# megapose6d/megapose6d

Measured on AMD Instinct MI355X. Metric: pose-hypotheses/sec (render+coarse+refine), 640×480, megapose-1.0-RGB, higher is better.
Workload: dtype f32 (results of fp32 arithmetic; the convolutions' multiplications run on the bf16 MFMA as EXACT piece products of the fp32 operands, fp32 accumulate)

## Files before the change

### include/mp_engine.h

```cpp
#ifndef MP_ENGINE_H
#define MP_ENGINE_H

#include <stddef.h>
#include <stdint.h>

#ifdef __cplusplus
extern "C" {
#endif

typedef void* mp_stream;

#define MP_OK 0
#define MP_ERR_INVALID (-22)
#define MP_ERR_NOMEM (-12)
#define MP_ERR_HIP (-5)

int mp_version(void);
const char* mp_last_error(void);
int mp_profile_begin(void);
int mp_profile_end(void);
int mp_profile_active(void);
int mp_profile_query(int idx, char* name, int name_len, int64_t* launches, double* total_ms, double* total_flops,
                     double* total_bytes);
int mp_profile_query_ex(int idx, char* name, int name_len, int64_t* launches, double* total_ms, double* total_flops,
// ... 110 lines not shown
const char* mp_conv2d_kernel_name(const mp_conv_desc* desc);

size_t mp_conv_bf16x9_packed_bytes(int Cin_p, int Cout, int KH, int KW);
int mp_conv_bf16x9_pack_weights(const float* h_w_oihw, int Cout, int Cin, int KH, int KW, int Cin_p, const float* h_scale ,
                                void* h_packed);
int mp_conv2d_bf16x9_nhwc(const mp_conv_desc* desc, const void* d_w_pieces, mp_stream stream);

size_t mp_conv_wino_packed_floats(int Cin_p, int Cout);
int mp_conv_wino_pack_weights(const float* h_w_oi33, int Cout, int Cin, int Cin_p, const float* h_scale , float* h_packed);
int mp_conv_wino_eligible(const mp_conv_desc* desc, int n_cu);
int mp_conv3x3_wino_nhwc(const mp_conv_desc* desc, const float* d_u, mp_stream stream);

size_t mp_conv_wino_bf16_packed_bytes(int Cin_p, int Cout);
int mp_conv_wino_bf16_pack_weights(const float* h_w_oi33, int Cout, int Cin, int Cin_p, const float* h_scale , void* h_packed);
int mp_conv3x3_wino_bf16_nhwc(const mp_conv_desc* desc, const void* d_u_pieces, mp_stream stream);

int mp_xrec_elements(int n_f32, int n_u8);
int mp_conv_stem_supported(int KS, int n_f32, int n_u8);
size_t mp_conv_stem_packed_bytes(int KS, int n_f32, int n_u8, int Cout);
int mp_conv_stem_pack_weights(const float* h_w_oihw, int Cout, int Cin, int KS, int n_f32, const float* h_scale ,
                              void* h_packed);
int mp_conv_stem_pack_weights_mask(const float* h_w_oihw, int Cout, int Cin, int KS, uint32_t f32_mask, const float* h_scale,
                                   void* h_packed);
int mp_conv_stem_xrec(const mp_conv_desc* desc, const void* d_packed, int n_f32, mp_stream stream);
int mp_conv_stem_xrec_pool(const mp_conv_desc* desc, const void* d_packed, int n_f32, float* d_ypool, int pool_border, mp_stream stream);

int mp_conv_stem_sparse_chunks(int KS, int n_f32, int n_u8);
size_t mp_conv_stem_sparse_packed_bytes(int KS, int n_f32, int n_u8, int Cout);
int mp_conv_stem_pack_weights_sparse(const float* h_w_oihw, int Cout, int Cin, int KS, int n_f32, const float* h_scale, void* h_packed);
int mp_conv_stem_xrec_sparse(const mp_conv_desc* desc, const void* d_packed, const void* d_packed_sparse, int n_f32,
// ... 151 lines not shown
```

### megapose6d_amd/_lib.py

```python
from __future__ import annotations

import ctypes as C
import os
from pathlib import Path

_HERE = Path(__file__).resolve().parent
LIB_PATH = _HERE / "libmp_engine.so"


class EngineError(RuntimeError):
    pass


class MeshDesc(C.Structure):
    _fields_ = [
        ("h_vertices", C.c_void_p),
        ("h_normals", C.c_void_p),
        ("h_colors", C.c_void_p),
        ("h_faces", C.c_void_p),
        ("n_vertices", C.c_int32),
        ("n_faces", C.c_int32),
    ]


# ... 85 lines not shown
    "mp_conv_pack_weights": (_i, [_vp, _i, _i, _i, _i, _i, _vp, _vp]),
    "mp_conv2d_nhwc": (_i, [C.POINTER(ConvDesc), _vp]),
    "mp_conv2d_plan": (_i, [C.POINTER(ConvDesc), _i, C.POINTER(C.c_int32)]),
    "mp_conv_bf16x9_packed_bytes": (_sz, [_i, _i, _i, _i]),
    "mp_conv_bf16x9_pack_weights": (_i, [_vp, _i, _i, _i, _i, _i, _vp, _vp]),
    "mp_conv2d_bf16x9_nhwc": (_i, [C.POINTER(ConvDesc), _vp, _vp]),
    "mp_conv2d_kernel_name": (C.c_char_p, [C.POINTER(ConvDesc)]),
    "mp_conv_wino_packed_floats": (_sz, [_i, _i]),
    "mp_conv_wino_pack_weights": (_i, [_vp, _i, _i, _i, _vp, _vp]),
    "mp_conv_wino_eligible": (_i, [C.POINTER(ConvDesc), _i]),
    "mp_conv3x3_wino_nhwc": (_i, [C.POINTER(ConvDesc), _vp, _vp]),
    "mp_conv_wino_stats": (_i, [C.POINTER(C.c_double), C.POINTER(C.c_double), _i]),
    "mp_conv_wino_bf16_packed_bytes": (_sz, [_i, _i]),
    "mp_conv_wino_bf16_pack_weights": (_i, [_vp, _i, _i, _i, _vp, _vp]),
    "mp_conv3x3_wino_bf16_nhwc": (_i, [C.POINTER(ConvDesc), _vp, _vp]),
    "mp_conv_wino_bf16_stats": (_i, [C.POINTER(C.c_double), C.POINTER(C.c_double), _i]),
    "mp_conv_wino_bf16_clock": (_i, [C.POINTER(C.c_double), C.POINTER(C.c_double), _i]),
    "mp_conv_wino_bf16_phases": (_i, [C.POINTER(C.c_double), C.POINTER(C.c_double)]),
    "mp_conv_wino_bf16_telemetry": (_i, [_i]),
    "mp_xrec_elements": (_i, [_i, _i]),
    "mp_conv_stem_supported": (_i, [_i, _i, _i]),
    "mp_conv_stem_packed_bytes": (_sz, [_i, _i, _i, _i]),
    "mp_conv_stem_pack_weights": (_i, [_vp, _i, _i, _i, _i, _vp, _vp]),
    "mp_conv_stem_pack_weights_mask": (_i, [_vp, _i, _i, _i, _u32, _vp, _vp]),
    "mp_conv_stem_sparse_chunks": (_i, [_i, _i, _i]),
    "mp_conv_stem_sparse_packed_bytes": (_sz, [_i, _i, _i, _i]),
    "mp_conv_stem_pack_weights_sparse": (_i, [_vp, _i, _i, _i, _i, _vp, _vp]),
    "mp_conv_stem_xrec_sparse": (_i, [C.POINTER(ConvDesc), _vp, _vp, _i, _vp, _vp, _i, _vp]),
    "mp_conv_stem_bg_stats": (_i, [C.POINTER(C.c_double), C.POINTER(C.c_double), _i]),
    "mp_conv_stem_xrec": (_i, [C.POINTER(ConvDesc), _vp, _i, _vp]),
# ... 81 lines not shown
```

### megapose6d_amd/csrc/backbone.hip

```cpp
#include <cmath>
#include <cstdlib>
#include <map>
#include <mutex>
#include <string>
#include <vector>

#include "common.h"

namespace mp {

struct ConvLayer {
  int Cin, Cin_p, Cout, K, stride, pad;
  float* d_w = nullptr;
  float* d_u = nullptr;
  void* d_ub = nullptr;
  void* d_wb = nullptr;
  float* d_b = nullptr;
};

struct BnAct {
  float* d_scale = nullptr;
  float* d_shift = nullptr;
};

// ... 113 lines not shown
    if (rc) return rc;
  }
  return MP_OK;
}

int make_bnact(mp_backbone* bb, const StateMap& sm, const std::string& bnkey, int C, BnAct* a) {
  std::vector<float> scale, shift;
  int rc = bn_affine(sm, bnkey, C, scale, shift);
  if (rc) return rc;
  rc = upload(bb, scale, &a->d_scale);
  if (rc) return rc;
  return upload(bb, shift, &a->d_shift);
}

constexpr size_t SPLITK_WS_FLOATS = 12u << 20;

int run_conv(const mp_backbone* bb, const ConvLayer& L, const float* x, int N, int H, int W, int in_border, float* y, int out_border,
             const float* res, int relu, float* y_act, const BnAct* act, hipStream_t s, float* splitk_ws = nullptr, bool x_f16 = false) {
  mp_conv_desc d;
  memset(&d, 0, sizeof(d));
  d.x_f16 = x_f16 ? 1 : 0;
  d.d_x = x; d.N = N; d.H = H; d.W = W; d.C = L.Cin_p; d.c_real = L.Cin; d.in_border = in_border;
  d.d_w = L.d_w; d.d_bias = L.d_b; d.Cout = L.Cout; d.KH = L.K; d.KW = L.K; d.stride = L.stride; d.pad = L.pad;
  d.d_y = y; d.out_border = out_border; d.d_residual = res; d.relu = relu;
  d.d_y_act = y_act;
  if (y_act) { d.d_act_scale = act->d_scale; d.d_act_shift = act->d_shift; }
  d.d_splitk_ws = splitk_ws;
  d.splitk_ws_floats = splitk_ws ? (int64_t)SPLITK_WS_FLOATS : 0;
  if ((L.d_u || L.d_ub || L.d_wb) && !x_f16) {
    static int n_cu = 0, n_cu_dev = -1, lds_ok = 0;
    int dev = 0;
    (void)hipGetDevice(&dev);
    if (n_cu_dev != dev) {
      if (hipDeviceGetAttribute(&n_cu, hipDeviceAttributeMultiprocessorCount, dev) != hipSuccess || n_cu <= 0) n_cu = 256;
      int lds = 0;
      lds_ok = hipDeviceGetAttribute(&lds, hipDeviceAttributeMaxSharedMemoryPerBlock, dev) == hipSuccess && lds >= 132 * 1024;
      n_cu_dev = dev;
    }
    if ((L.d_u || L.d_ub) && lds_ok && mp_conv_wino_eligible(&d, n_cu))
      return L.d_ub ? mp_conv3x3_wino_bf16_nhwc(&d, L.d_ub, s) : mp_conv3x3_wino_nhwc(&d, L.d_u, s);
    if (L.d_wb) {
      int32_t plan[5] = {0, 1, 0, 0, 0};
      const int rc = mp_conv2d_plan(&d, n_cu, plan);
      if (rc) return rc;
      if (plan[0] != 1) return mp_conv2d_bf16x9_nhwc(&d, L.d_wb, s);
    }
  }
  return mp_conv2d_nhwc(&d, s);
}

inline size_t align_up(size_t v, size_t a) { return (v + a - 1) / a * a; }
inline size_t buf_floats(int N, int H, int W, int C) { return (size_t)N * (H + 2) * (W + 2) * C + (size_t)(W + 3) * C + 64; }

struct Geometry {
  int h1, w1;
// ... 2 lines not shown

Geometry geometry(const mp_backbone* bb, int h, int w) {
  Geometry g;
  g.h1 = (h + 2 * bb->stem.pad - bb->stem.K) / 2 + 1;
  g.w1 = (w + 2 * bb->stem.pad - bb->stem.K) / 2 + 1;
  g.hs[0] = (g.h1 + 2 - 3) / 2 + 1;
  g.ws[0] = (g.w1 + 2 - 3) / 2 + 1;
  for (int s = 1; s < 4; ++s) {
    g.hs[s] = (g.hs[s - 1] + 2 - 3) / 2 + 1;
    g.ws[s] = (g.ws[s - 1] + 2 - 3) / 2 + 1;
  }
  return g;
}


}

extern "C" int mp_backbone_create(int kind, int c_in, int head_kind, int n_head_out, const mp_named_tensor* st, int n_tensors,
                                  mp_backbone** out) {
  return mp_backbone_create_wide(kind, 1, c_in, head_kind, n_head_out, st, n_tensors, out);
}

extern "C" int mp_backbone_create_wide(int kind, int width, int c_in, int head_kind, int n_head_out, const mp_named_tensor* st, int n_tensors,
                                       mp_backbone** out) {
  MP_REQUIRE(out && st && n_tensors > 0, "mp_backbone_create: bad arguments");
  MP_REQUIRE(kind >= 0 && kind <= 2, "mp_backbone_create: unknown backbone kind %d", kind);
  MP_REQUIRE(width >= 1 && width <= 8 && (width == 1 || kind != MP_BACKBONE_VANILLA_RESNET34),
             "mp_backbone_create: width multiplier %d (1..8, WideResNets only: training/pose_models_cfg.py:114-116)", width);
  MP_REQUIRE(c_in >= 1 && c_in <= 512, "mp_backbone_create: bad c_in %d", c_in);
  StateMap sm;
// ... 286 lines not shown
```

### megapose6d_amd/csrc/conv_wino_bf16.hip

```cpp
#include <atomic>
#include <cstdlib>
#include <mutex>
#include <vector>

#include "bf16x9_split.h"
#include "wino_common.h"

namespace mp {

typedef __bf16 bf16x8 __attribute__((ext_vector_type(8)));
typedef float f32x2 __attribute__((ext_vector_type(2)));


__device__ __forceinline__ unsigned pack_hi16(unsigned e1, unsigned e0) { return __builtin_amdgcn_perm(e1, e0, 0x07060302u); }

__device__ __forceinline__ float f4c(const float4& v, int c) { return c == 0 ? v.x : c == 1 ? v.y : c == 2 ? v.z : v.w; }
__device__ constexpr int WB_PA[9] = {2, 1, 2, 0, 1, 2, 0, 1, 0}, WB_PB[9] = {2, 2, 1, 2, 1, 0, 1, 0, 0};

constexpr int UB_F_BYTES = 2 * 3 * 1024;
constexpr int UB_STEP_BYTES = 16 * UB_F_BYTES;
constexpr size_t WB_LDS_BYTES = (size_t)4 * 2 * WT * 72 * sizeof(float);
static_assert(WB_LDS_BYTES >= WINO_LDS_BYTES && WB_LDS_BYTES <= 160 * 1024, "LDS budget of conv3x3_wino_bf16x9");

__device__ unsigned long long g_wb_clk[6];
#ifdef MP_WINO_PHASES
__device__ unsigned long long g_wb_phase[10];
#define WB_PHASE(K, T0) if (ph_sample) atomicAdd(&g_wb_phase[K], __builtin_readcyclecounter() - (T0));
#else
#define WB_PHASE(K, T0)
#endif

template <int DIAG, bool RES, bool ACT, bool PERSIST = false>
__global__ __launch_bounds__(256) __attribute__((amdgpu_waves_per_eu(1, 1))) void conv3x3_wino_bf16x9(WinoParams p) {
  extern __shared__ __attribute__((aligned(16))) float smem[];
  float* Vs = smem;
  int* tile_tab = (int*)(smem + 4 * 2 * WT * WCOUT);

  unsigned long long clk_start = __builtin_readcyclecounter();
  const int tid = threadIdx.x, lane = tid & 63;
#ifdef MP_WINO_PHASES
  const bool ph_sample = (blockIdx.x & 63) == 0 && threadIdx.x == 0;
#endif
  const int wave = __builtin_amdgcn_readfirstlane(tid >> 6);
  const __amdgpu_buffer_rsrc_t x_rsrc = __builtin_amdgcn_make_buffer_rsrc((void*)p.x, 0, -1, 0x00020000);
  const int row_bytes = p.Wp * p.C * 4, pix_bytes = p.C * 4;
  const int u_voff = lane * 16;
  const int ptile = tid >> 2, pc4 = tid & 3;
  float4 patch[4][4];
  int unit = (int)blockIdx.x;
  const int n_units = PERSIST ? p.n_units : (int)gridDim.x;
  int cb, tile0, x_voff;
  __amdgpu_buffer_rsrc_t u_rsrc;
#define WB_UNIT_INDICES(U)                                                                               \
  {                                                                                                      \
    const int wg_ = xcd_remap((U), n_units);                                                             \
    const int tg_ = (int)wino_fastdiv((unsigned)wg_, (unsigned)p.n_cblocks, p.mg_cb, p.sh_cb);           \
    cb = wg_ - tg_ * p.n_cblocks;                                                                        \
    tile0 = tg_ * WT;                                                                                    \
    const unsigned char* ub_ = reinterpret_cast<const unsigned char*>(p.u) + (size_t)cb * p.n_steps * UB_STEP_BYTES + (size_t)(4 * wave) * UB_F_BYTES;  \
    u_rsrc = __builtin_amdgcn_make_buffer_rsrc((void*)ub_, 0, -1, 0x00020000);                            \
    int t_ = tile0 + ptile;                                                                              \
    t_ = t_ < p.n_tiles ? t_ : p.n_tiles - 1;                                                            \
    const int r_ = (int)wino_fastdiv((unsigned)t_, (unsigned)p.tiles_x, p.mg_tx, p.sh_tx), tx_ = t_ - r_ * p.tiles_x;   \
    const int n_ = (int)wino_fastdiv((unsigned)r_, (unsigned)p.tiles_y, p.mg_ty, p.sh_ty), ty_ = r_ - n_ * p.tiles_y;   \
    const size_t pix_ = ((size_t)n_ * p.Hp + (size_t)(2 * ty_ + p.in_off)) * p.Wp + (size_t)(2 * tx_ + p.in_off);  \
    x_voff = (int)((pix_ * p.C + pc4 * 4) * sizeof(float));                                               \
  }
  float* vw = Vs + ptile * WCK + ((pc4 ^ ((ptile >> 2) & 3)) * 4);



  f32x16 acc[4][2][2];
  const int ns = p.n_steps;
  u32x4 Ua[2][3], Ub[2][3];
  u32x4 AA[2][3], AB[2][3];
  float4 raw[2][2];
  unsigned sm0, sm1, sm2, sm3;
  float sr0, sr1, sr2, sr3, sq0, sq1, sq2, sq3;
  float4 trw[4], tplane;
  if (DIAG & (7 | 32 | 64 | 128)) {
    _Pragma("unroll") for (int i = 0; i < 2; ++i)
      _Pragma("unroll") for (int q = 0; q < 3; ++q) { AA[i][q] = AB[i][q] = Ua[i][q] = Ub[i][q] = u32x4{0x3f803f80u, 0x3f803f80u, 0x3f803f80u, 0x3f803f80u}; }
    _Pragma("unroll") for (int a = 0; a < 4; ++a) { trw[a] = make_float4(0.f, 0.f, 0.f, 0.f);
      _Pragma("unroll") for (int bb = 0; bb < 4; ++bb) patch[a][bb] = make_float4(1.f, 1.f, 1.f, 1.f); }
    tplane = make_float4(0.f, 0.f, 0.f, 0.f);
    sm0 = sm1 = sm2 = sm3 = 0u; sr0 = sr1 = sr2 = sr3 = sq0 = sq1 = sq2 = sq3 = 0.f;
  }
#define WB_SB __builtin_amdgcn_sched_barrier(0);
// ... 90 lines not shown
  const int fo_lo = ((2 * (lane >> 5)) ^ fsw) * 4, fo_hi = ((2 * (lane >> 5) + 1) ^ fsw) * 4;

  float4 pnext[4][4];
#define WB_UNIT_REQUESTS() \
  _Pragma("unroll") for (int a = 0; a < 4; ++a) \
    _Pragma("unroll") for (int bb = 0; bb < 4; ++bb) { WB_LOAD_PATCH1(a, bb, 0) } \
  WB_SB \
  if (tid < WT) { \
    const int t = tile0 + tid; \
    int off = -1, bits = 0; \
    if (t < p.n_tiles) { \
      const int r = (int)wino_fastdiv((unsigned)t, (unsigned)p.tiles_x, p.mg_tx, p.sh_tx), tx = t - r * p.tiles_x; \
      const int n = (int)wino_fastdiv((unsigned)r, (unsigned)p.tiles_y, p.mg_ty, p.sh_ty), ty = r - n * p.tiles_y; \
      off = ((n * p.Hop + 2 * ty + p.out_border) * p.Wop + 2 * tx + p.out_border) * p.Cout; \
      bits = ((2 * ty + 1 < p.Ho) ? 1 : 0) | ((2 * tx + 1 < p.Wo) ? 2 : 0); \
    } \
    tile_tab[2 * tid] = off; \
    tile_tab[2 * tid + 1] = bits; \
  } \
  { \
    const u32x4 z4 = {0u, 0u, 0u, 0u}; \
    _Pragma("unroll") for (int fi = 0; fi < 4; ++fi) \
      _Pragma("unroll") for (int i = 0; i < 2; ++i) \
        _Pragma("unroll") for (int j = 0; j < 2; ++j) \
          asm volatile("s_nop 1\n\tv_mfma_f32_32x32x16_bf16 %0, %1, %1, 0" : "=a"(acc[fi][i][j]) : "v"(z4)); \
  } \
  WB_SB
#define WB_UNIT_TABLE() \
  if (tid < WT) { \
    const int t = tile0 + tid; \
    int off = -1, bits = 0; \
    if (t < p.n_tiles) { \
      const int r = (int)wino_fastdiv((unsigned)t, (unsigned)p.tiles_x, p.mg_tx, p.sh_tx), tx = t - r * p.tiles_x; \
      const int n = (int)wino_fastdiv((unsigned)r, (unsigned)p.tiles_y, p.mg_ty, p.sh_ty), ty = r - n * p.tiles_y; \
      off = ((n * p.Hop + 2 * ty + p.out_border) * p.Wop + 2 * tx + p.out_border) * p.Cout; \
      bits = ((2 * ty + 1 < p.Ho) ? 1 : 0) | ((2 * tx + 1 < p.Wo) ? 2 : 0); \
    } \
    tile_tab[2 * tid] = off; \
    tile_tab[2 * tid + 1] = bits; \
  }
  WB_UNIT_INDICES(unit)
  WB_UNIT_REQUESTS()
  for (;;) {
  _Pragma("unroll") for (int k = 0; k < 6; ++k) { WB_LOAD_U1(Ua, 0, 0, k) }
  WB_SB
  WB_PHASE(0, clk_start)
#define WB_TR_ROW(A, VW) WB_TR_T(A, 0) WB_TR_T(A, 1) WB_TR_T(A, 2) WB_TR_T(A, 3) WB_TR_P(0) WB_TR_W(A, 0, VW) WB_TR_P(1) WB_TR_W(A, 1, VW) WB_TR_P(2) WB_TR_W(A, 2, VW) WB_TR_P(3) WB_TR_W(A, 3, VW)
  WB_TR_ROW(0, vw) WB_PHASE(1, clk_start)
  WB_SB
  const int cs1 = (ns > 1 ? 1 : 0) * (WCK * 4);
#define WB_PN(K) WB_SB pnext[(K) >> 2][(K) & 3] = buf4(x_rsrc, x_voff, cs1 + ((K) >> 2) * row_bytes + ((K) & 3) * pix_bytes); WB_SB
// ... 3 lines not shown
  WB_TR_ROW_PN(1, vw, 0) WB_PN(5) WB_TR_ROW_PN(2, vw, 6) WB_TR_ROW_PN(3, vw, 11)
#undef WB_TR_ROW_PN
#undef WB_PN
  WB_PHASE(2, clk_start)
  _Pragma("unroll") for (int a = 0; a < 4; ++a)
    _Pragma("unroll") for (int bb = 0; bb < 4; ++bb) patch[a][bb] = pnext[a][bb];
  __syncthreads();
  WB_PHASE(3, clk_start)
  constexpr unsigned WOOB = 0xFFFFFFF0u;
  int2 ttab[4];
  _Pragma("unroll") for (int it = 0; it < 4; ++it) ttab[it] = *reinterpret_cast<const int2*>(tile_tab + 2 * (it * 16 + (tid >> 4)));
  WB_READ_RAW1(vr, 0, 0) WB_READ_RAW1(vr, 0, 1) WB_READ_RAW1(vr, 0, 2) WB_READ_RAW1(vr, 0, 3)
#define WB_SPLIT4(AN, I, H) WB_SP0(AN, I, H) WB_SP1(I, H) WB_SP2(AN, I, H) WB_SP3() WB_SP4(AN, I, H)
  WB_SPLIT4(AA, 0, 0) WB_SPLIT4(AA, 0, 1) WB_SPLIT4(AA, 1, 0) WB_SPLIT4(AA, 1, 1)
  WB_READ_RAW1(vr, 1, 0) WB_READ_RAW1(vr, 1, 1) WB_READ_RAW1(vr, 1, 2) WB_READ_RAW1(vr, 1, 3)
  const int n = cb * WCOUT + (tid & 15) * 4;
  unsigned voff[4][4];
  {
    const int e_row = p.Wop * p.Cout * 4, e_pix = p.Cout * 4;
    _Pragma("unroll") for (int it = 0; it < 4; ++it) {
      const int off = ttab[it].x, bits = ttab[it].y;
      const unsigned base = (unsigned)(off + n) * 4u;
      const bool t_ok = off >= 0;
      voff[it][0] = t_ok ? base : WOOB;
      voff[it][1] = (t_ok && (bits & 2)) ? base + (unsigned)e_pix : WOOB;
      voff[it][2] = (t_ok && (bits & 1)) ? base + (unsigned)e_row : WOOB;
      voff[it][3] = (t_ok && (bits & 3) == 3) ? base + (unsigned)(e_row + e_pix) : WOOB;
    }
  }
  const int out_bytes = p.out_bytes;
  const __amdgpu_buffer_rsrc_t r_res = __builtin_amdgcn_make_buffer_rsrc((void*)p.residual, 0, (RES && p.residual) ? out_bytes : 0, 0x00020000);
  u32x4 res[4][4];

#ifdef MP_WINO_PERMUTE
// ... 178 lines not shown
#undef WB_TR_W
#undef WB_TR_P
#undef WB_TR_ROW
#undef WB_TR_T
#undef WB_F4ASM
#undef WB_OP_SUB
#undef WB_OP_ADD
#undef WB_LOAD_PATCH1
#undef WB_LOAD_U1
#undef WB_SB
#undef WB_UNIT_TABLE
#undef WB_UNIT_REQUESTS
#undef WB_UNIT_INDICES
}

}

using namespace mp;

extern "C" size_t mp_conv_wino_bf16_packed_bytes(int Cin_p, int Cout) { return (size_t)(Cout / WCOUT) * (Cin_p / WCK) * UB_STEP_BYTES; }

extern "C" int mp_conv_wino_bf16_pack_weights(const float* w, int Cout, int Cin, int Cin_p, const float* scale, void* packed_bytes) {
  MP_REQUIRE(w && packed_bytes && Cin_p >= Cin && Cin_p % WCK == 0 && Cout % WCOUT == 0,
             "mp_conv_wino_bf16_pack_weights: bad arguments (Cin_p %% 16, Cout %% 64)");
  static const double G[4][3] = {{1, 0, 0}, {0.5, 0.5, 0.5}, {0.5, -0.5, 0.5}, {0, 0, 1}};
  const int n_steps = Cin_p / WCK;
  unsigned short* out = (unsigned short*)packed_bytes;
  memset(out, 0, mp_conv_wino_bf16_packed_bytes(Cin_p, Cout));
  for (int n = 0; n < Cout; ++n) {
    const double s = scale ? (double)scale[n] : 1.0;
// ... 52 lines not shown
#endif

extern "C" int mp_conv_wino_bf16_clock(double* shader_mhz, double* cycles_per_step, int reset) {
  unsigned long long h[6] = {0, 0, 0, 0, 0, 0};
  MP_CHECK_HIP(hipDeviceSynchronize());
  MP_CHECK_HIP(hipMemcpyFromSymbol(h, HIP_SYMBOL(g_wb_clk), sizeof(h)));
  if (shader_mhz) *shader_mhz = h[1] ? 100.0 * (double)h[0] / (double)h[1] : 0.0;
  if (cycles_per_step) *cycles_per_step = h[2] ? (double)h[0] / (double)h[2] : 0.0;
  if (reset) {
    const unsigned long long z[6] = {0, 0, 0, 0, 0, 0};
    MP_CHECK_HIP(hipMemcpyToSymbol(HIP_SYMBOL(g_wb_clk), z, sizeof(z)));
  }
  return MP_OK;
}

extern "C" int mp_conv3x3_wino_bf16_nhwc(const mp_conv_desc* d, const void* d_u_pieces, mp_stream stream) {
  MP_REQUIRE(d && d->d_x && d_u_pieces && (d->d_y || d->d_y_act), "mp_conv3x3_wino_bf16_nhwc: null pointer");
  MP_REQUIRE(d->KH == 3 && d->KW == 3 && d->stride == 1 && d->pad == 1, "mp_conv3x3_wino_bf16_nhwc: 3x3 / stride 1 / pad 1 only");
  MP_REQUIRE(d->C % WCK == 0 && d->Cout % WCOUT == 0 && d->in_border >= 1, "mp_conv3x3_wino_bf16_nhwc: C %% 16, Cout %% 64, in_border >= 1");
  MP_REQUIRE(!d->d_y_act || (d->d_act_scale && d->d_act_shift), "mp_conv3x3_wino_bf16_nhwc: y_act needs scale/shift");
  WinoParams p;
  p.x = d->d_x; p.u = (const float*)d_u_pieces; p.bias = d->d_bias; p.residual = d->d_residual; p.act_scale = d->d_act_scale; p.act_shift = d->d_act_shift;
  p.y = d->d_y; p.y_act = d->d_y_act;
  p.N = d->N; p.Ho = d->H; p.Wo = d->W;
  p.Hp = d->H + 2 * d->in_border; p.Wp = d->W + 2 * d->in_border; p.C = d->C;
  p.in_off = d->in_border - 1;
  p.Cout = d->Cout;
  p.Hop = d->H + 2 * d->out_border; p.Wop = d->W + 2 * d->out_border; p.out_border = d->out_border;
  p.tiles_x = (d->W + 1) / 2; p.tiles_y = (d->H + 1) / 2;
  const long n_tiles = (long)d->N * p.tiles_x * p.tiles_y;
  const long in_bytes = ((long)d->N * p.Hp + 2) * p.Wp * p.C * 4, out_elems = (long)d->N * p.Hop * p.Wop * d->Cout;
// ... 2 lines not shown
  p.n_tiles = (int)n_tiles;
  p.n_chunks = d->C / 8;
  p.n_steps = d->C / WCK;
  wino_fastdiv_make((unsigned)p.tiles_x, &p.mg_tx, &p.sh_tx);
  wino_fastdiv_make((unsigned)p.tiles_y, &p.mg_ty, &p.sh_ty);
  p.relu = d->relu;
  p.n_cblocks = d->Cout / WCOUT;
  wino_fastdiv_make((unsigned)p.n_cblocks, &p.mg_cb, &p.sh_cb);
  int dev = 0;
  MP_CHECK_HIP(hipGetDevice(&dev));
  static int attr_dev = -1;
  if (attr_dev != dev) {
#define WB_ATTR(...) MP_CHECK_HIP(hipFuncSetAttribute((const void*)conv3x3_wino_bf16x9<__VA_ARGS__>, hipFuncAttributeMaxDynamicSharedMemorySize, (int)WB_LDS_BYTES));
    WB_ATTR(0, false, false) WB_ATTR(0, true, false) WB_ATTR(0, false, true) WB_ATTR(0, true, true)
    WB_ATTR(0, false, false, true) WB_ATTR(0, true, false, true) WB_ATTR(0, false, true, true) WB_ATTR(0, true, true, true)
#ifdef MP_CONV_EXPERIMENTS
    WB_ATTR(1, true, true) WB_ATTR(2, true, true) WB_ATTR(4, true, true) WB_ATTR(7, true, true) WB_ATTR(8, true, true) WB_ATTR(16, true, true)
    WB_ATTR(32, true, true) WB_ATTR(64, true, true) WB_ATTR(128, true, true)
#endif
#undef WB_ATTR
    attr_dev = dev;
  }
  const long n_wg = ((n_tiles + WT - 1) / WT) * p.n_cblocks;
  hipStream_t s = (hipStream_t)stream;
  const double c_real = d->c_real > 0 ? d->c_real : d->C;
  const double direct = 2.0 * 9.0 * (double)d->N * d->H * d->W * c_real * d->Cout;
  const double executed = 9.0 * 2.0 * 16.0 * (double)n_tiles * c_real * d->Cout;
  {
    std::lock_guard<std::mutex> lock(g_wb_mu);
    g_wb_direct += direct;
    g_wb_executed += executed;
  }
  p.telemetry = g_wb_telemetry.load(std::memory_order_relaxed);
  ProfScope prof("conv3x3_wino_bf16x9<64t,64c>", direct, 4.0 * ((double)d->N * d->H * d->W * (d->C + d->Cout)) + 6.0 * 16.0 * d->C * d->Cout, s, executed, 2500.0);
  const dim3 grid((unsigned)n_wg), block(256);
  static const int persist_env = getenv("MP_WINO_PERSIST") ? atoi(getenv("MP_WINO_PERSIST")) : 1;
  static int n_cu = 0;
  if (!n_cu) { hipDeviceProp_t prop; MP_CHECK_HIP(hipGetDeviceProperties(&prop, dev)); n_cu = prop.multiProcessorCount; }
  p.n_units = (int)n_wg;
  bool launched = false;
#ifdef MP_CONV_EXPERIMENTS
  const int diag = getenv("MP_WINO_DIAG") ? atoi(getenv("MP_WINO_DIAG")) : 0;
#define WB_DIAG_LAUNCH(D) if (diag == D) { hipLaunchKernelGGL((conv3x3_wino_bf16x9<D, true, true>), grid, block, WB_LDS_BYTES, s, p); launched = true; }
  WB_DIAG_LAUNCH(1) WB_DIAG_LAUNCH(2) WB_DIAG_LAUNCH(4) WB_DIAG_LAUNCH(7) WB_DIAG_LAUNCH(8) WB_DIAG_LAUNCH(16) WB_DIAG_LAUNCH(32) WB_DIAG_LAUNCH(64) WB_DIAG_LAUNCH(128)
#undef WB_DIAG_LAUNCH
#endif
  if (launched) {
  } else if (persist_env && n_wg > n_cu) {
    const dim3 pgrid((unsigned)n_cu);
    if (d->d_residual && d->d_y_act) hipLaunchKernelGGL((conv3x3_wino_bf16x9<0, true, true, true>), pgrid, block, WB_LDS_BYTES, s, p);
    else if (d->d_residual) hipLaunchKernelGGL((conv3x3_wino_bf16x9<0, true, false, true>), pgrid, block, WB_LDS_BYTES, s, p);
    else if (d->d_y_act) hipLaunchKernelGGL((conv3x3_wino_bf16x9<0, false, true, true>), pgrid, block, WB_LDS_BYTES, s, p);
    else hipLaunchKernelGGL((conv3x3_wino_bf16x9<0, false, false, true>), pgrid, block, WB_LDS_BYTES, s, p);
  } else if (d->d_residual && d->d_y_act) hipLaunchKernelGGL((conv3x3_wino_bf16x9<0, true, true>), grid, block, WB_LDS_BYTES, s, p);
  else if (d->d_residual) hipLaunchKernelGGL((conv3x3_wino_bf16x9<0, true, false>), grid, block, WB_LDS_BYTES, s, p);
  else if (d->d_y_act) hipLaunchKernelGGL((conv3x3_wino_bf16x9<0, false, true>), grid, block, WB_LDS_BYTES, s, p);
  else hipLaunchKernelGGL((conv3x3_wino_bf16x9<0, false, false>), grid, block, WB_LDS_BYTES, s, p);
  MP_CHECK_HIP(hipGetLastError());
  return MP_OK;
}
```

### megapose6d_amd/csrc/wino_common.h

```cpp
#pragma once
#include "common.h"

namespace mp {

typedef float f32x16 __attribute__((ext_vector_type(16)));
typedef unsigned u32x4 __attribute__((ext_vector_type(4)));

constexpr int WT = 64;
constexpr int WCK = 16;
constexpr int WCOUT = 64;

struct WinoParams {
  const float* __restrict__ x;
  const float* __restrict__ u;
  const float* __restrict__ bias;
  const float* __restrict__ residual;
  const float* __restrict__ act_scale;
  const float* __restrict__ act_shift;
  float* __restrict__ y;
  float* __restrict__ y_act;
  int N, Ho, Wo;
  int Hp, Wp, C;
  int in_off;
  int Cout;
  int Hop, Wop, out_border;
  int tiles_x, tiles_y, n_tiles;
  int n_chunks;
  int n_steps;
  int relu;
  int n_cblocks;
  int out_bytes;
  unsigned mg_tx, sh_tx, mg_ty, sh_ty, mg_cb, sh_cb;
  int n_units;
  int telemetry;
};

__device__ __forceinline__ float4 buf4(__amdgpu_buffer_rsrc_t r, int voff, int soff) {
  const u32x4 v = __builtin_amdgcn_raw_buffer_load_b128(r, voff, soff, 0);
  return make_float4(__uint_as_float(v.x), __uint_as_float(v.y), __uint_as_float(v.z), __uint_as_float(v.w));
}

static inline void wino_fastdiv_make(unsigned d, unsigned* M, unsigned* s) {
  unsigned l = 0;
  while ((1ull << l) < d) ++l;
  *M = (unsigned)(((1ull << 32) * ((1ull << l) - d)) / d + 1);
  *s = l;
}
__device__ __forceinline__ unsigned wino_fastdiv(unsigned t, unsigned d, unsigned M, unsigned s) {
  const unsigned t1 = __umulhi(t, M);
// ... 9 lines not shown
```

### megapose6d_amd/engine.py

```python
from __future__ import annotations

import ctypes as C
from typing import Dict, List, Optional, Sequence, Tuple

import numpy as np
import torch

from . import _lib
from ._lib import ConvDesc, EngineError, Lights, MeshDesc, NamedTensor, check

RASTER_NORMALS = 1
RASTER_DEPTH = 2
RASTER_NORMALS_GL = 4
RASTER_MSAA4 = 16
RASTER_F16 = 32
RASTER_XREC = 64

BACKBONE_KINDS = {"vanilla_resnet34": 0, "resnet34": 1, "resnet18": 2}


def _stream() -> int:
    return torch.cuda.current_stream().cuda_stream


# ... 322 lines not shown
                      bias: Optional[torch.Tensor], Cout: int, y: Optional[torch.Tensor], out_border: int,
                      residual: Optional[torch.Tensor] = None, relu: bool = False, y_act: Optional[torch.Tensor] = None,
                      act_scale: Optional[torch.Tensor] = None, act_shift: Optional[torch.Tensor] = None) -> None:
    d = ConvDesc()
    d.d_x, d.N, d.H, d.W, d.C, d.in_border = x.data_ptr(), N, H, W, Cp, in_border
    d.d_bias = _ptr(bias)
    d.Cout, d.KH, d.KW, d.stride, d.pad = Cout, 3, 3, 1, 1
    d.d_y, d.out_border, d.d_residual, d.relu = _ptr(y), out_border, _ptr(residual), int(relu)
    d.d_y_act, d.d_act_scale, d.d_act_shift = _ptr(y_act), _ptr(act_scale), _ptr(act_shift)
    if u_packed.dtype == torch.uint8:
        check(_lib.load().mp_conv3x3_wino_bf16_nhwc(C.byref(d), u_packed.data_ptr(), _stream()))
        return
    check(_lib.load().mp_conv3x3_wino_nhwc(C.byref(d), u_packed.data_ptr(), _stream()))


def conv_wino_eligible(N: int, H: int, W: int, Cp: int, in_border: int, Cout: int, out_border: int, n_cu: int) -> bool:
    d = ConvDesc()
    d.N, d.H, d.W, d.C, d.in_border = N, H, W, Cp, in_border
    d.Cout, d.KH, d.KW, d.stride, d.pad = Cout, 3, 3, 1, 1
    d.out_border = out_border
    return bool(_lib.load().mp_conv_wino_eligible(C.byref(d), n_cu))


def conv_wino_bf16_pack_weights(w_oihw: np.ndarray, cin_p: int, scale: Optional[np.ndarray] = None) -> np.ndarray:
    lib = _lib.load()
    w = np.ascontiguousarray(w_oihw, dtype=np.float32)
    Cout, Cin, KH, KW = w.shape
    assert KH == 3 and KW == 3
    out = np.empty(lib.mp_conv_wino_bf16_packed_bytes(cin_p, Cout), dtype=np.uint8)
    sc = None if scale is None else np.ascontiguousarray(scale, dtype=np.float32)
# ... 554 lines not shown
```

Before: 2263.

## Split the Winograd bf16 conv tail wave across K slices with a reduce pass

Adds a split-K path for the partial last round of workgroups in the bf16 Winograd 3x3 conv. Full rounds run as before, and the leftover tail units are spread over 2–4 K-range slices that write partial sums to the split-K scratch. A separate reduce kernel then applies bias, residual, ReLU and the BN activation. A cost model chooses the slice count, so that idle CUs during the tail are filled, at the price of an extra launch and the scratch traffic.

```diff
diff --git a/include/mp_engine.h b/include/mp_engine.h
--- a/include/mp_engine.h
+++ b/include/mp_engine.h
@@ -148,6 +148,8 @@
 size_t mp_conv_wino_bf16_packed_bytes(int Cin_p, int Cout);
 int mp_conv_wino_bf16_pack_weights(const float* h_w_oi33, int Cout, int Cin, int Cin_p, const float* h_scale , void* h_packed);
 int mp_conv3x3_wino_bf16_nhwc(const mp_conv_desc* desc, const void* d_u_pieces, mp_stream stream);
+int mp_conv3x3_wino_bf16_split_nhwc(const mp_conv_desc* desc, const void* d_u_pieces, int n_main_units, int n_slices, mp_stream stream);
+int mp_conv_wino_plan(int units, int steps, int n_cu, int32_t* out3);
 
 int mp_xrec_elements(int n_f32, int n_u8);
 int mp_conv_stem_supported(int KS, int n_f32, int n_u8);
diff --git a/megapose6d_amd/_lib.py b/megapose6d_amd/_lib.py
--- a/megapose6d_amd/_lib.py
+++ b/megapose6d_amd/_lib.py
@@ -123,6 +123,8 @@
     "mp_conv_wino_bf16_packed_bytes": (_sz, [_i, _i]),
     "mp_conv_wino_bf16_pack_weights": (_i, [_vp, _i, _i, _i, _vp, _vp]),
     "mp_conv3x3_wino_bf16_nhwc": (_i, [C.POINTER(ConvDesc), _vp, _vp]),
+    "mp_conv3x3_wino_bf16_split_nhwc": (_i, [C.POINTER(ConvDesc), _vp, _i, _i, _vp]),
+    "mp_conv_wino_plan": (_i, [_i, _i, _i, C.POINTER(C.c_int32)]),
     "mp_conv_wino_bf16_stats": (_i, [C.POINTER(C.c_double), C.POINTER(C.c_double), _i]),
     "mp_conv_wino_bf16_clock": (_i, [C.POINTER(C.c_double), C.POINTER(C.c_double), _i]),
     "mp_conv_wino_bf16_phases": (_i, [C.POINTER(C.c_double), C.POINTER(C.c_double)]),
diff --git a/megapose6d_amd/csrc/backbone.hip b/megapose6d_amd/csrc/backbone.hip
--- a/megapose6d_amd/csrc/backbone.hip
+++ b/megapose6d_amd/csrc/backbone.hip
@@ -151,6 +151,31 @@
 }
 
 constexpr size_t SPLITK_WS_FLOATS = 12u << 20;
+
+struct WinoPlan {
+  int rounds, tail_units, slices;
+};
+constexpr double WINO_STEP_CYC = 5.9e3;
+constexpr double WINO_FIXED_WALK_CYC = 10.2e3;
+constexpr double WINO_FIXED_ALONE_CYC = 12.8e3;
+constexpr double WINO_BYTES_PER_CYC = 2.5e3;
+constexpr double WINO_BOUNDARY_CYC = 4.3e3;
+constexpr double WINO_UNIT_BYTES = 64.0 * 4 * 64 * 4;
+
+WinoPlan plan_wino(int units, int steps, int n_cu) {
+  WinoPlan pl = {units / n_cu, units % n_cu, 1};
+  const int t = pl.tail_units;
+  if (t == 0) return pl;
+  double best = (pl.rounds > 0 ? WINO_FIXED_WALK_CYC : WINO_FIXED_ALONE_CYC) + steps * WINO_STEP_CYC;
+  for (int S = 2; S <= 4 && S <= steps; S *= 2) {
+    if ((double)t * S * WINO_UNIT_BYTES > (double)SPLITK_WS_FLOATS * sizeof(float)) break;
+    const int piece_rounds = (t * S + n_cu - 1) / n_cu, piece_steps = (steps + S - 1) / S;
+    const double cost = piece_rounds * (WINO_FIXED_ALONE_CYC + piece_steps * WINO_STEP_CYC) + t * WINO_UNIT_BYTES * (2 * S + 2) / WINO_BYTES_PER_CYC +
+                        (pl.rounds > 0 ? 2 : 1) * WINO_BOUNDARY_CYC;
+    if (cost < best) { best = cost; pl.slices = S; }
+  }
+  return pl;
+}
 
 int run_conv(const mp_backbone* bb, const ConvLayer& L, const float* x, int N, int H, int W, int in_border, float* y, int out_border,
              const float* res, int relu, float* y_act, const BnAct* act, hipStream_t s, float* splitk_ws = nullptr, bool x_f16 = false) {
@@ -174,8 +199,16 @@
       lds_ok = hipDeviceGetAttribute(&lds, hipDeviceAttributeMaxSharedMemoryPerBlock, dev) == hipSuccess && lds >= 132 * 1024;
       n_cu_dev = dev;
     }
-    if ((L.d_u || L.d_ub) && lds_ok && mp_conv_wino_eligible(&d, n_cu))
-      return L.d_ub ? mp_conv3x3_wino_bf16_nhwc(&d, L.d_ub, s) : mp_conv3x3_wino_nhwc(&d, L.d_u, s);
+    if ((L.d_u || L.d_ub) && lds_ok && mp_conv_wino_eligible(&d, n_cu)) {
+      if (!L.d_ub) return mp_conv3x3_wino_nhwc(&d, L.d_u, s);
+      static const int tail_split = getenv("MP_WINO_TAIL_SPLIT") ? atoi(getenv("MP_WINO_TAIL_SPLIT")) : 1;
+      if (tail_split && splitk_ws) {
+        const long tiles = (long)N * ((H + 1) / 2) * ((W + 1) / 2);
+        const WinoPlan pl = plan_wino((int)(((tiles + 63) / 64) * (L.Cout / 64)), L.Cin_p / 16, n_cu);
+        if (pl.slices > 1) return mp_conv3x3_wino_bf16_split_nhwc(&d, L.d_ub, pl.rounds * n_cu, pl.slices, s);
+      }
+      return mp_conv3x3_wino_bf16_nhwc(&d, L.d_ub, s);
+    }
     if (L.d_wb) {
       int32_t plan[5] = {0, 1, 0, 0, 0};
       const int rc = mp_conv2d_plan(&d, n_cu, plan);
@@ -208,6 +241,13 @@
 }
 
 
+}
+
+extern "C" int mp_conv_wino_plan(int units, int steps, int n_cu, int32_t* out3) {
+  MP_REQUIRE(out3 && units >= 1 && steps >= 1 && n_cu >= 1, "mp_conv_wino_plan: bad arguments");
+  const WinoPlan pl = plan_wino(units, steps, n_cu);
+  out3[0] = pl.rounds; out3[1] = pl.tail_units; out3[2] = pl.slices;
+  return MP_OK;
 }
 
 extern "C" int mp_backbone_create(int kind, int c_in, int head_kind, int n_head_out, const mp_named_tensor* st, int n_tensors,
diff --git a/megapose6d_amd/csrc/conv_wino_bf16.hip b/megapose6d_amd/csrc/conv_wino_bf16.hip
--- a/megapose6d_amd/csrc/conv_wino_bf16.hip
+++ b/megapose6d_amd/csrc/conv_wino_bf16.hip
@@ -30,8 +30,11 @@
 #define WB_PHASE(K, T0)
 #endif
 
+constexpr int WB_KRANGE = 256;
 template <int DIAG, bool RES, bool ACT, bool PERSIST = false>
 __global__ __launch_bounds__(256) __attribute__((amdgpu_waves_per_eu(1, 1))) void conv3x3_wino_bf16x9(WinoParams p) {
+  constexpr bool KRANGE = (DIAG & WB_KRANGE) != 0;
+  static_assert(!KRANGE || (!RES && !ACT && !PERSIST), "the K-range launch is the plain one-workgroup-per-unit instance");
   extern __shared__ __attribute__((aligned(16))) float smem[];
   float* Vs = smem;
   int* tile_tab = (int*)(smem + 4 * 2 * WT * WCOUT);
@@ -53,11 +56,13 @@
   __amdgpu_buffer_rsrc_t u_rsrc;
 #define WB_UNIT_INDICES(U)                                                                               \
   {                                                                                                      \
-    const int wg_ = xcd_remap((U), n_units);                                                             \
+    int wg_ = xcd_remap((U), n_units);                                                                   \
+    if constexpr (KRANGE) wg_ = kr_unit;                                                                 \
     const int tg_ = (int)wino_fastdiv((unsigned)wg_, (unsigned)p.n_cblocks, p.mg_cb, p.sh_cb);           \
     cb = wg_ - tg_ * p.n_cblocks;                                                                        \
     tile0 = tg_ * WT;                                                                                    \
     const unsigned char* ub_ = reinterpret_cast<const unsigned char*>(p.u) + (size_t)cb * p.n_steps * UB_STEP_BYTES + (size_t)(4 * wave) * UB_F_BYTES;  \
+    if constexpr (KRANGE) ub_ += (size_t)kr_s0 * UB_STEP_BYTES;                                          \
     u_rsrc = __builtin_amdgcn_make_buffer_rsrc((void*)ub_, 0, -1, 0x00020000);                            \
     int t_ = tile0 + ptile;                                                                              \
     t_ = t_ < p.n_tiles ? t_ : p.n_tiles - 1;                                                            \
@@ -65,13 +70,21 @@
     const int n_ = (int)wino_fastdiv((unsigned)r_, (unsigned)p.tiles_y, p.mg_ty, p.sh_ty), ty_ = r_ - n_ * p.tiles_y;   \
     const size_t pix_ = ((size_t)n_ * p.Hp + (size_t)(2 * ty_ + p.in_off)) * p.Wp + (size_t)(2 * tx_ + p.in_off);  \
     x_voff = (int)((pix_ * p.C + pc4 * 4) * sizeof(float));                                               \
+    if constexpr (KRANGE) x_voff += kr_s0 * (WCK * (int)sizeof(float));                                  \
   }
   float* vw = Vs + ptile * WCK + ((pc4 ^ ((ptile >> 2) & 3)) * 4);
 
 
 
   f32x16 acc[4][2][2];
-  const int ns = p.n_steps;
+  int kr_unit = 0, kr_s0 = 0, kr_s1 = 0;
+  if constexpr (KRANGE) {
+    const int sl = (int)blockIdx.x / p.split_units;
+    kr_unit = p.unit0 + ((int)blockIdx.x - sl * p.split_units);
+    kr_s0 = sl * p.n_steps / p.n_slices;
+    kr_s1 = (sl + 1) * p.n_steps / p.n_slices;
+  }
+  const int ns = KRANGE ? kr_s1 - kr_s0 : p.n_steps;
   u32x4 Ua[2][3], Ub[2][3];
   u32x4 AA[2][3], AB[2][3];
   float4 raw[2][2];
@@ -192,6 +205,7 @@
       const int n = (int)wino_fastdiv((unsigned)r, (unsigned)p.tiles_y, p.mg_ty, p.sh_ty), ty = r - n * p.tiles_y; \
       off = ((n * p.Hop + 2 * ty + p.out_border) * p.Wop + 2 * tx + p.out_border) * p.Cout; \
       bits = ((2 * ty + 1 < p.Ho) ? 1 : 0) | ((2 * tx + 1 < p.Wo) ? 2 : 0); \
+      if constexpr (KRANGE) { off = ((int)blockIdx.x * WT + tid) * (4 * WCOUT); bits = 3; }    \
     } \
     tile_tab[2 * tid] = off; \
     tile_tab[2 * tid + 1] = bits; \
@@ -213,6 +227,7 @@
       const int n = (int)wino_fastdiv((unsigned)r, (unsigned)p.tiles_y, p.mg_ty, p.sh_ty), ty = r - n * p.tiles_y; \
       off = ((n * p.Hop + 2 * ty + p.out_border) * p.Wop + 2 * tx + p.out_border) * p.Cout; \
       bits = ((2 * ty + 1 < p.Ho) ? 1 : 0) | ((2 * tx + 1 < p.Wo) ? 2 : 0); \
+      if constexpr (KRANGE) { off = ((int)blockIdx.x * WT + tid) * (4 * WCOUT); bits = 3; }    \
     } \
     tile_tab[2 * tid] = off; \
     tile_tab[2 * tid + 1] = bits; \
@@ -246,10 +261,10 @@
 #define WB_SPLIT4(AN, I, H) WB_SP0(AN, I, H) WB_SP1(I, H) WB_SP2(AN, I, H) WB_SP3() WB_SP4(AN, I, H)
   WB_SPLIT4(AA, 0, 0) WB_SPLIT4(AA, 0, 1) WB_SPLIT4(AA, 1, 0) WB_SPLIT4(AA, 1, 1)
   WB_READ_RAW1(vr, 1, 0) WB_READ_RAW1(vr, 1, 1) WB_READ_RAW1(vr, 1, 2) WB_READ_RAW1(vr, 1, 3)
-  const int n = cb * WCOUT + (tid & 15) * 4;
+  const int n = KRANGE ? (tid & 15) * 4 : cb * WCOUT + (tid & 15) * 4;
   unsigned voff[4][4];
   {
-    const int e_row = p.Wop * p.Cout * 4, e_pix = p.Cout * 4;
+    const int e_row = KRANGE ? 2 * WCOUT * 4 : p.Wop * p.Cout * 4, e_pix = KRANGE ? WCOUT * 4 : p.Cout * 4;
     _Pragma("unroll") for (int it = 0; it < 4; ++it) {
       const int off = ttab[it].x, bits = ttab[it].y;
       const unsigned base = (unsigned)(off + n) * 4u;
@@ -458,6 +473,47 @@
 #undef WB_UNIT_INDICES
 }
 
+__global__ __launch_bounds__(256) void conv_wino_split_reduce(WinoParams p, const float* __restrict__ part) {
+  const long idx = (long)blockIdx.x * blockDim.x + threadIdx.x;
+  if (idx >= (long)p.split_units * (WT * 4 * (WCOUT / 4))) return;
+  const int c4 = (int)(idx & 15), px = (int)(idx >> 4) & 3, tl = (int)(idx >> 6) & (WT - 1), ul = (int)(idx >> 12);
+  const int unit = p.unit0 + ul;
+  const int tg = unit / p.n_cblocks, cb = unit - tg * p.n_cblocks;
+  const int t = tg * WT + tl;
+  if (t >= p.n_tiles) return;
+  const int r = t / p.tiles_x, tx = t - r * p.tiles_x;
+  const int ni = r / p.tiles_y, ty = r - ni * p.tiles_y;
+  const int ho = 2 * ty + (px >> 1), wo = 2 * tx + (px & 1);
+  if (ho >= p.Ho || wo >= p.Wo) return;
+  const size_t slice_floats = (size_t)p.split_units * (WT * 4 * WCOUT);
+  const float* q = part + (size_t)idx * 4;
+  float4 v = *reinterpret_cast<const float4*>(q);
+  for (int z = 1; z < p.n_slices; ++z) {
+    const float4 w = *reinterpret_cast<const float4*>(q + (size_t)z * slice_floats);
+    v.x += w.x; v.y += w.y; v.z += w.z; v.w += w.w;
+  }
+  const int n = cb * WCOUT + c4 * 4;
+  const size_t off = (((size_t)ni * p.Hop + ho + p.out_border) * p.Wop + wo + p.out_border) * p.Cout + n;
+  if (p.bias) {
+    const float4 b = *reinterpret_cast<const float4*>(p.bias + n);
+    v.x += b.x; v.y += b.y; v.z += b.z; v.w += b.w;
+  }
+  if (p.residual) {
+    const float4 rr = *reinterpret_cast<const float4*>(p.residual + off);
+    v.x += rr.x; v.y += rr.y; v.z += rr.z; v.w += rr.w;
+  }
+  const float relu_floor = p.relu != 0 ? 0.f : __builtin_nanf("");
+  v.x = fmaxf(v.x, relu_floor); v.y = fmaxf(v.y, relu_floor); v.z = fmaxf(v.z, relu_floor); v.w = fmaxf(v.w, relu_floor);
+  if (p.y) *reinterpret_cast<float4*>(p.y + off) = v;
+  if (p.y_act) {
+    const float4 sc = *reinterpret_cast<const float4*>(p.act_scale + n), sh = *reinterpret_cast<const float4*>(p.act_shift + n);
+    float4 a;
+    a.x = fmaxf(fmaf(v.x, sc.x, sh.x), 0.f); a.y = fmaxf(fmaf(v.y, sc.y, sh.y), 0.f);
+    a.z = fmaxf(fmaf(v.z, sc.z, sh.z), 0.f); a.w = fmaxf(fmaf(v.w, sc.w, sh.w), 0.f);
+    *reinterpret_cast<float4*>(p.y_act + off) = a;
+  }
+}
+
 }
 
 using namespace mp;
@@ -540,7 +596,7 @@
   return MP_OK;
 }
 
-extern "C" int mp_conv3x3_wino_bf16_nhwc(const mp_conv_desc* d, const void* d_u_pieces, mp_stream stream) {
+static int wino_bf16_launch(const mp_conv_desc* d, const void* d_u_pieces, long n_main, int n_slices, mp_stream stream) {
   MP_REQUIRE(d && d->d_x && d_u_pieces && (d->d_y || d->d_y_act), "mp_conv3x3_wino_bf16_nhwc: null pointer");
   MP_REQUIRE(d->KH == 3 && d->KW == 3 && d->stride == 1 && d->pad == 1, "mp_conv3x3_wino_bf16_nhwc: 3x3 / stride 1 / pad 1 only");
   MP_REQUIRE(d->C % WCK == 0 && d->Cout % WCOUT == 0 && d->in_border >= 1, "mp_conv3x3_wino_bf16_nhwc: C %% 16, Cout %% 64, in_border >= 1");
@@ -573,6 +629,7 @@
 #define WB_ATTR(...) MP_CHECK_HIP(hipFuncSetAttribute((const void*)conv3x3_wino_bf16x9<__VA_ARGS__>, hipFuncAttributeMaxDynamicSharedMemorySize, (int)WB_LDS_BYTES));
     WB_ATTR(0, false, false) WB_ATTR(0, true, false) WB_ATTR(0, false, true) WB_ATTR(0, true, true)
     WB_ATTR(0, false, false, true) WB_ATTR(0, true, false, true) WB_ATTR(0, false, true, true) WB_ATTR(0, true, true, true)
+    MP_CHECK_HIP(hipFuncSetAttribute((const void*)conv3x3_wino_bf16x9<WB_KRANGE, false, false>, hipFuncAttributeMaxDynamicSharedMemorySize, (int)WB_LDS_BYTES));
 #ifdef MP_CONV_EXPERIMENTS
     WB_ATTR(1, true, true) WB_ATTR(2, true, true) WB_ATTR(4, true, true) WB_ATTR(7, true, true) WB_ATTR(8, true, true) WB_ATTR(16, true, true)
     WB_ATTR(32, true, true) WB_ATTR(64, true, true) WB_ATTR(128, true, true)
@@ -580,7 +637,17 @@
 #undef WB_ATTR
     attr_dev = dev;
   }
-  const long n_wg = ((n_tiles + WT - 1) / WT) * p.n_cblocks;
+  const long n_units_all = ((n_tiles + WT - 1) / WT) * p.n_cblocks;
+  const long n_wg = n_main < 0 ? n_units_all : n_main;
+  const long n_tail = n_units_all - n_wg;
+  const size_t part_bytes = (size_t)n_tail * n_slices * (WT * 4 * WCOUT * sizeof(float));
+  if (n_main >= 0) {
+    MP_REQUIRE(n_main < n_units_all && n_slices >= 2 && n_slices <= p.n_steps,
+               "mp_conv3x3_wino_bf16_split_nhwc: %ld of %ld units in the plain launch, %d slices of %d K steps", n_main, n_units_all, n_slices, p.n_steps);
+    MP_REQUIRE(d->d_splitk_ws && part_bytes <= (size_t)d->splitk_ws_floats * sizeof(float) && part_bytes < (1u << 31),
+               "mp_conv3x3_wino_bf16_split_nhwc: split-K scratch %zu < %zu bytes", (size_t)d->splitk_ws_floats * sizeof(float), part_bytes);
+  }
+  p.unit0 = 0; p.split_units = 0; p.n_slices = 1;
   hipStream_t s = (hipStream_t)stream;
   const double c_real = d->c_real > 0 ? d->c_real : d->C;
   const double direct = 2.0 * 9.0 * (double)d->N * d->H * d->W * c_real * d->Cout;
@@ -591,6 +658,7 @@
     g_wb_executed += executed;
   }
   p.telemetry = g_wb_telemetry.load(std::memory_order_relaxed);
+  {
   ProfScope prof("conv3x3_wino_bf16x9<64t,64c>", direct, 4.0 * ((double)d->N * d->H * d->W * (d->C + d->Cout)) + 6.0 * 16.0 * d->C * d->Cout, s, executed, 2500.0);
   const dim3 grid((unsigned)n_wg), block(256);
   static const int persist_env = getenv("MP_WINO_PERSIST") ? atoi(getenv("MP_WINO_PERSIST")) : 1;
@@ -604,7 +672,7 @@
   WB_DIAG_LAUNCH(1) WB_DIAG_LAUNCH(2) WB_DIAG_LAUNCH(4) WB_DIAG_LAUNCH(7) WB_DIAG_LAUNCH(8) WB_DIAG_LAUNCH(16) WB_DIAG_LAUNCH(32) WB_DIAG_LAUNCH(64) WB_DIAG_LAUNCH(128)
 #undef WB_DIAG_LAUNCH
 #endif
-  if (launched) {
+  if (launched || n_wg == 0) {
   } else if (persist_env && n_wg > n_cu) {
     const dim3 pgrid((unsigned)n_cu);
     if (d->d_residual && d->d_y_act) hipLaunchKernelGGL((conv3x3_wino_bf16x9<0, true, true, true>), pgrid, block, WB_LDS_BYTES, s, p);
@@ -616,5 +684,28 @@
   else if (d->d_y_act) hipLaunchKernelGGL((conv3x3_wino_bf16x9<0, false, true>), grid, block, WB_LDS_BYTES, s, p);
   else hipLaunchKernelGGL((conv3x3_wino_bf16x9<0, false, false>), grid, block, WB_LDS_BYTES, s, p);
   MP_CHECK_HIP(hipGetLastError());
+  if (n_tail == 0) return MP_OK;
+  WinoParams q = p;
+  q.bias = nullptr; q.residual = nullptr; q.act_scale = nullptr; q.act_shift = nullptr; q.y_act = nullptr; q.relu = 0;
+  q.y = d->d_splitk_ws;
+  q.out_bytes = (int)part_bytes;
+  q.unit0 = (int)n_wg; q.split_units = (int)n_tail; q.n_slices = n_slices;
+  hipLaunchKernelGGL((conv3x3_wino_bf16x9<WB_KRANGE, false, false>), dim3((unsigned)(n_tail * n_slices)), block, WB_LDS_BYTES, s, q);
+  MP_CHECK_HIP(hipGetLastError());
+  }
+  p.unit0 = (int)n_wg; p.split_units = (int)n_tail; p.n_slices = n_slices;
+  const double px4 = (double)n_tail * (WT * 4 * (WCOUT / 4));
+  ProfScope prof("conv_wino_split_reduce", 0.0, 16.0 * px4 * (n_slices + 1 + (d->d_residual ? 1 : 0) + (d->d_y && d->d_y_act ? 1 : 0)), s);
+  hipLaunchKernelGGL(conv_wino_split_reduce, dim3((unsigned)ceil_div((long)px4, 256L)), dim3(256), 0, s, p, (const float*)d->d_splitk_ws);
+  MP_CHECK_HIP(hipGetLastError());
   return MP_OK;
 }
+
+extern "C" int mp_conv3x3_wino_bf16_nhwc(const mp_conv_desc* d, const void* d_u_pieces, mp_stream stream) {
+  return wino_bf16_launch(d, d_u_pieces, -1, 1, stream);
+}
+
+extern "C" int mp_conv3x3_wino_bf16_split_nhwc(const mp_conv_desc* d, const void* d_u_pieces, int n_main_units, int n_slices, mp_stream stream) {
+  MP_REQUIRE(n_main_units >= 0, "mp_conv3x3_wino_bf16_split_nhwc: n_main_units %d", n_main_units);
+  return wino_bf16_launch(d, d_u_pieces, n_main_units, n_slices, stream);
+}
diff --git a/megapose6d_amd/csrc/wino_common.h b/megapose6d_amd/csrc/wino_common.h
--- a/megapose6d_amd/csrc/wino_common.h
+++ b/megapose6d_amd/csrc/wino_common.h
@@ -33,6 +33,7 @@
   unsigned mg_tx, sh_tx, mg_ty, sh_ty, mg_cb, sh_cb;
   int n_units;
   int telemetry;
+  int unit0, split_units, n_slices;
 };
 
 __device__ __forceinline__ float4 buf4(__amdgpu_buffer_rsrc_t r, int voff, int soff) {
diff --git a/megapose6d_amd/engine.py b/megapose6d_amd/engine.py
--- a/megapose6d_amd/engine.py
+++ b/megapose6d_amd/engine.py
@@ -360,6 +360,28 @@
     check(_lib.load().mp_conv3x3_wino_nhwc(C.byref(d), u_packed.data_ptr(), _stream()))
 
 
+def conv3x3_wino_bf16_split_nhwc(x: torch.Tensor, N: int, H: int, W: int, Cp: int, in_border: int, u_pieces: torch.Tensor,
+                                 bias: Optional[torch.Tensor], Cout: int, y: Optional[torch.Tensor], out_border: int, n_main_units: int,
+                                 n_slices: int, scratch: torch.Tensor, residual: Optional[torch.Tensor] = None, relu: bool = False,
+                                 y_act: Optional[torch.Tensor] = None, act_scale: Optional[torch.Tensor] = None,
+                                 act_shift: Optional[torch.Tensor] = None) -> None:
+    d = ConvDesc()
+    d.d_x, d.N, d.H, d.W, d.C, d.in_border = x.data_ptr(), N, H, W, Cp, in_border
+    d.d_bias = _ptr(bias)
+    d.Cout, d.KH, d.KW, d.stride, d.pad = Cout, 3, 3, 1, 1
+    d.d_y, d.out_border, d.d_residual, d.relu = _ptr(y), out_border, _ptr(residual), int(relu)
+    d.d_y_act, d.d_act_scale, d.d_act_shift = _ptr(y_act), _ptr(act_scale), _ptr(act_shift)
+    assert scratch.dtype == torch.float32
+    d.d_splitk_ws, d.splitk_ws_floats = scratch.data_ptr(), scratch.numel()
+    check(_lib.load().mp_conv3x3_wino_bf16_split_nhwc(C.byref(d), u_pieces.data_ptr(), n_main_units, n_slices, _stream()))
+
+
+def conv_wino_plan(units: int, steps: int, n_cu: int) -> Dict[str, int]:
+    out = (C.c_int32 * 3)()
+    check(_lib.load().mp_conv_wino_plan(units, steps, n_cu, out))
+    return dict(zip(("rounds", "tail_units", "slices"), out))
+
+
 def conv_wino_eligible(N: int, H: int, W: int, Cp: int, in_border: int, Cout: int, out_border: int, n_cu: int) -> bool:
     d = ConvDesc()
     d.N, d.H, d.W, d.C, d.in_border = N, H, W, Cp, in_border
```

Result: no change. 2258 (-0.2%).
